# carkod/binquant

Measured on AMD Instinct MI355X. Metric: symbol-candles/s for full indicator set (14 fp64 columns), higher is better.
Workload: dtype f64; 1 GPU; configs[3]: 100000 symbols x 10000 candles, symbol-sharded over 1 GPU(s) (100000 symbols x 10000 candles on rank 0); symbols=100000, symbols_per_gpu=100000, candles=10000, parallelism=symbol-sharded x1, no data-path collective

## Files before the change

### binquant_amd/csrc/bq_context.hip

```cpp
#include "bq_context.h"
#include "binquant_amd.h"

#include <string.h>

namespace bq {

constexpr int CX_NW = 4;
constexpr int CX_NT = CX_NW * WAVE;
constexpr int CX_K = CTX_K;
constexpr int CX_TT = WAVE * CX_K;
constexpr int CX_HS = 20;
constexpr int CX_RS = CX_HS + CX_TT;
constexpr int CX_Q = CX_RS / CX_K;
static_assert(CX_HS % CX_K == 0 && CX_RS % CX_K == 0, "ring shape");
#define CXS(i) ((((i) & (CX_K - 1)) * CX_Q) + ((i) >> 2))
constexpr int CX_ATR = 14;
constexpr int CX_BB = 20;

constexpr int CNT_VALID = 0, CNT_ADV = 3, CNT_DEC = 6, CNT_A20 = 9, CNT_A50 = 12;

struct CtxArgs {
  const double* h;
  const double* l;
  const double* c;
  int64_t S, ld_in;
  int T, M;
  int vin;
  FeatEma E;
  int lag20, lag50;
  double* gsum[4];
  uint16_t* gcnt;
  int64_t ld_g;
  double* last[BQ_NUM_FEATURES];
  double* feat[BQ_NUM_FEATURES];
  int64_t ld_f;
  int vout;
};

__device__ __forceinline__ void wave_sync() {
  __builtin_amdgcn_fence(__ATOMIC_RELEASE, "wavefront");
  __builtin_amdgcn_wave_barrier();
  __builtin_amdgcn_fence(__ATOMIC_ACQUIRE, "wavefront");
}

__device__ __forceinline__ double cx_rcp(double b) { return rcp_nr(fabs(b)); }
__device__ __forceinline__ double cx_mul_rcp(double a, double b, double r) { return b < 0.0 ? -(a * r) : a * r; }
__device__ __forceinline__ double cx_div(double a, double b) { return cx_mul_rcp(a, b, cx_rcp(b)); }

template <bool DIV, bool RING, bool FEAT = false, int MC = 0>
__global__ __launch_bounds__(CX_NT, 3) void context_partials_kernel(const CtxArgs A) {
  __shared__ double sTr[CX_NW][CX_RS], sC[CX_NW][CX_RS];
  __shared__ double sR[2][4][CX_TT];
  __shared__ uint16_t sN[2][CX_TT];
  __shared__ float sD[RING ? CX_NW : 1][RING ? 3 * CX_TT : 1];

  const int lane = threadIdx.x & (WAVE - 1), w = threadIdx.x / WAVE;
  const int64_t grp = blockIdx.x;
  const int64_t sym = grp * CX_NW + w;
  const bool live = sym < A.S;
  const int64_t row = live ? sym : A.S - 1;
  const int T = A.T, M = MC > 0 ? MC : A.M;
  const double* __restrict__ rH = A.h + row * A.ld_in;
  const double* __restrict__ rL = A.l + row * A.ld_in;
  const double* __restrict__ rC = A.c + row * A.ld_in;
  double* __restrict__ trr = sTr[w];
  double* __restrict__ cr = sC[w];
  const bool vin = A.vin != 0;
  const int WB = M < CX_BB ? M : CX_BB;

  if (lane < CX_HS) {
    trr[CXS(lane)] = 0.0;
    cr[CXS(lane)] = qnan();
  }
  double c1c = qnan(), c2c = qnan(), hc = qnan(), lc = qnan();
  int rcC = -1, rtC = -1;
  double ecar[2] = {0.0, 0.0}, lcar[2] = {0.0, 0.0};
  double lpow[2], rpow[2];
#pragma unroll
  for (int e = 0; e < 2; ++e) {
    lpow[e] = pow_bits<6>(A.E.apow[e], lane);
    rpow[e] = pow_bits<5>(A.E.apow[e], (lane & 15) + 1);
  }
  wave_sync();

  for (int t0 = 0; t0 < T; t0 += CX_TT) {
    const int tb = t0 + CX_K * lane, qb = CX_HS + CX_K * lane;
    double h[CX_K], l[CX_K], c[CX_K], xl[CX_K];
    load4<double2>(rH, tb, T, vin, h);
    load4<double2>(rL, tb, T, vin, l);
    load4<double2>(rC, tb, T, vin, c);
    if (!RING && (A.lag20 || A.lag50)) {
#pragma unroll
      for (int k = 0; k < CX_K; ++k) {
        const int s = tb + k - (M - 1);
        xl[k] = (s >= 0 && s < T) ? rC[s] : 0.0;
      }
    }

    double p1 = dpp_f64<DPP_WAVE_SHR1>(c[CX_K - 1]);
    double p2 = dpp_f64<DPP_WAVE_SHR1>(c[CX_K - 2]);
    double ph = dpp_f64<DPP_WAVE_SHR1>(h[CX_K - 1]);
    double pl = dpp_f64<DPP_WAVE_SHR1>(l[CX_K - 1]);
    if (lane == 0) {
      p1 = c1c;
      p2 = c2c;
      ph = hc;
      pl = lc;
    }
    double tr[CX_K];
    int lcc[CX_K], lct[CX_K];
    {
      double pcv = p1, ptr = true_range(ph, pl, p2), cp = p1;
      int rc = -1, rt = -1;
#pragma unroll
      for (int k = 0; k < CX_K; ++k) {
        const int t = tb + k;
        tr[k] = true_range(h[k], l[k], cp);
        if (t == 0 || c[k] != pcv) rc = t;
        if (t == 0 || tr[k] != ptr) rt = t;
        lcc[k] = rc;
        lct[k] = rt;
        pcv = c[k];
        ptr = tr[k];
        cp = c[k];
      }
    }
#pragma unroll
    for (int k = 0; k < CX_K; ++k) {
      cr[CXS(qb + k)] = c[k];
      trr[CXS(qb + k)] = tr[k];
    }
    {
      const int ic = wave_scan_max_dpp(lcc[CX_K - 1] + 1, lane) - 1;
      const int it = wave_scan_max_dpp(lct[CX_K - 1] + 1, lane) - 1;
      const int a = dpp_i32<DPP_WAVE_SHR1>(ic + 1) - 1, b = dpp_i32<DPP_WAVE_SHR1>(it + 1) - 1;
      const int ec = max(lane == 0 ? -1 : a, rcC), et = max(lane == 0 ? -1 : b, rtC);
#pragma unroll
      for (int k = 0; k < CX_K; ++k) {
        lcc[k] = max(lcc[k], ec);
        lct[k] = max(lct[k], et);
      }
    }
    double Y[2][CX_K], D[2][CX_K];
#pragma unroll
    for (int e = 0; e < 2; ++e) {
      const double al = A.E.alpha[e], om = A.E.om[e], dn = A.E.den[e];
      {
        double y = 0.0;
#pragma unroll
        for (int k = 0; k < CX_K; ++k) y = (tb + k == 0) ? c[k] : fma(A.E.lin_a[e], y, A.E.lin_b[e] * c[k]);
        const double inc = wave_scan_affine_dpp_rp(y, A.E.apow[e], rpow[e], lane);
        const double ex = dpp_f64<DPP_WAVE_SHR1>(inc);
        double v = lane == 0 ? ecar[e] : fma(lpow[e], ecar[e], ex);
#pragma unroll
        for (int k = 0; k < CX_K; ++k) {
          const double x = c[k];
          if (tb + k == 0) v = x;
          else if (v != x) v = DIV ? (om * v + al * x) / dn : om * v + al * x;
          Y[e][k] = v;
        }
        ecar[e] = readlane_f64(v, WAVE - 1);
      }
      const bool lag = !RING && (e == 0 ? A.lag20 : A.lag50);
#pragma unroll
      for (int k = 0; k < CX_K; ++k) D[e][k] = 0.0;
      if (lag) {
        const int s0 = tb - (M - 1);
        double y = 0.0;
#pragma unroll
        for (int k = 0; k < CX_K; ++k) y = (s0 + k == 0) ? xl[k] : fma(A.E.lin_a[e], y, A.E.lin_b[e] * xl[k]);
        const double inc = wave_scan_affine_dpp_rp(y, A.E.apow[e], rpow[e], lane);
        const double ex = dpp_f64<DPP_WAVE_SHR1>(inc);
        double v = lane == 0 ? lcar[e] : fma(lpow[e], lcar[e], ex);
#pragma unroll
        for (int k = 0; k < CX_K; ++k) {
          const int s = s0 + k;
          const double x = xl[k];
          if (s == 0) v = x;
          else if (s > 0 && v != x) v = DIV ? (om * v + al * x) / dn : om * v + al * x;
          D[e][k] = v - x;
        }
        lcar[e] = readlane_f64(v, WAVE - 1);
      }
    }
    if (RING) {
      float* dr = sD[w];
      const int dslot = ((t0 / CX_TT) % 3) * CX_TT;
#pragma unroll
      for (int k = 0; k < CX_K; ++k) dr[dslot + CX_K * lane + k] = (float)(Y[1][k] - c[k]);
    }
    wave_sync();
    if (RING) {
      const float* dr = sD[w];
      int r = ((t0 / CX_TT) % 3) * CX_TT + CX_K * lane - (M - 1);
      r += r < 0 ? 3 * CX_TT : 0;
#pragma unroll
      for (int k = 0; k < CX_K; ++k) {
        const int q = r + k >= 3 * CX_TT ? r + k - 3 * CX_TT : r + k;
        D[1][k] = (double)dr[q];
      }
    }

    double atr[CX_K], mid[CX_K], sd[CX_K];
    if (tb >= CX_BB - 1 && WB == CX_BB) {
      {
        double a[CX_ATR - 1];
#pragma unroll
        for (int i = 0; i < CX_ATR - 1; ++i) a[i] = trr[CXS(qb - (CX_ATR - 1) + i)];
        double Sx = 0.0;
#pragma unroll
        for (int i = 0; i < CX_ATR - 1; ++i) Sx += a[i];
#pragma unroll
        for (int k = 0; k < CX_K; ++k) {
          Sx = k == 0 ? Sx + tr[0] : (Sx + tr[k]) - a[k - 1];
          atr[k] = div_count(Sx < 0.0 ? 0.0 : Sx, (double)CX_ATR, 1.0 / CX_ATR);
        }
      }
      {
        const double r = c[0];
        double d0[CX_K - 1];
        double s1 = 0.0, s2 = 0.0;
#pragma unroll
        for (int i = 0; i < CX_BB - 1; ++i) {
          const double d = cr[CXS(qb - (CX_BB - 1) + i)] - r;
          if (i < CX_K - 1) d0[i] = d;
          s1 += d;
          s2 = fma(d, d, s2);
        }
#pragma unroll
        for (int k = 0; k < CX_K; ++k) {
          const double dn = c[k] - r;
          if (k == 0) {
            s1 += dn;
            s2 = fma(dn, dn, s2);
          } else {
            const double dol = d0[k - 1];
            s1 = (s1 + dn) - dol;
            s2 = fma(-dol, dol, fma(dn, dn, s2));
          }
          const double m1 = s1 * (1.0 / CX_BB);
          const double var = fma(-m1, s1, s2) * (1.0 / CX_BB);
          mid[k] = r + m1;
          sd[k] = sqrt_nr(var > 0.0 ? var : 0.0);
        }
      }
    } else {
#pragma unroll
      for (int k = 0; k < CX_K; ++k) {
        const int t = tb + k, q = qb + k;
        const int n = min(t + 1, M);
        const int ma = min(CX_ATR, n), mb = min(WB, n);
        double Sx = 0.0;
        for (int i = q - ma + 1; i <= q; ++i) Sx += trr[CXS(i)];
        atr[k] = (Sx < 0.0 ? 0.0 : Sx) / (double)ma;
        double m = 0.0;
        for (int i = q - mb + 1; i <= q; ++i) m += cr[CXS(i)];
        m = m / (double)mb;
        double acc = 0.0;
        for (int i = q - mb + 1; i <= q; ++i) {
          const double d = cr[CXS(i)] - m;
          acc = fma(d, d, acc);
        }
        mid[k] = m;
        sd[k] = sqrt(acc / (double)mb);
      }
    }
    double fr[CX_K], fe20[CX_K], fe50[CX_K], ftr[CX_K], fap[CX_K], fbw[CX_K];
    double rc[CX_K + 1];
    rc[0] = cx_rcp(p1);
#pragma unroll
    for (int k = 0; k < CX_K; ++k) rc[k + 1] = cx_rcp(c[k]);
#pragma unroll
    for (int k = 0; k < CX_K; ++k) {
      const int t = tb + k;
      const int n = min(t + 1, M);
      if (n < 2) {
        fr[k] = fe20[k] = fe50[k] = ftr[k] = fap[k] = fbw[k] = qnan();
        continue;
      }
      const double cl = c[k];
      const double prev = k > 0 ? c[k - 1] : p1;
      double e20 = Y[0][k], e50 = Y[1][k];
      if (t + 1 > M) {
        e20 = e20 - A.E.corr[0] * D[0][k];
        e50 = e50 - A.E.corr[1] * D[1][k];
      }
      const double a = lct[k] <= t - min(CX_ATR, n) + 1 ? tr[k] : atr[k];
      double m = mid[k], s = sd[k];
      if (lcc[k] <= t - min(WB, n) + 1) {
        m = cl;
        s = 0.0;
      }
      const double up = m + (2.0 * s), lo = m - (2.0 * s);
      fr[k] = prev == 0.0 ? 0.0 : cx_mul_rcp(cl - prev, prev, rc[k]);
      fe20[k] = e20;
      fe50[k] = e50;
      ftr[k] = e50 != 0.0 ? cx_div(e20 - e50, e50 < 0.0 ? -e50 : e50) : 0.0;
      fap[k] = cl != 0.0 ? cx_mul_rcp(a, cl, rc[k + 1]) : 0.0;
      fbw[k] = m != 0.0 ? cx_div(up - lo, m < 0.0 ? -m : m) : 0.0;
    }
    if constexpr (FEAT) {
      if (live) {
        const int64_t orow = sym * A.ld_f;
        const bool vo = A.vout != 0, whole = t0 + CX_TT <= T;
        const double* const cols[BQ_NUM_FEATURES] = {fr, fe20, fe50, ftr, fap, fbw};
#pragma unroll
        for (int f = 0; f < BQ_NUM_FEATURES; ++f)
          if (A.feat[f]) {
            double v[CX_K];
#pragma unroll
            for (int k = 0; k < CX_K; ++k) v[k] = cols[f][k];
            store_lines<CX_K>(A.feat[f] + orow, tb, T, vo, v, whole);
          }
      }
    } else {
    if (live && tb <= T - 1 && T - 1 < tb + CX_K) {
#pragma unroll
      for (int k = 0; k < CX_K; ++k) {
        if (tb + k != T - 1) continue;
        const double v[BQ_NUM_FEATURES] = {fr[k], fe20[k], fe50[k], ftr[k], fap[k], fbw[k]};
#pragma unroll
        for (int f = 0; f < BQ_NUM_FEATURES; ++f)
          if (A.last[f]) A.last[f][sym] = v[f];
      }
    }

    double cs[4][CX_K];
    unsigned cn[CX_K];
#pragma unroll
    for (int k = 0; k < CX_K; ++k) {
      const double r = fr[k];
      const bool ok = live && tb + k < T && r == r;
      cn[k] = ok ? ((1u << CNT_VALID) | ((r > 0.0 ? 1u : 0u) << CNT_ADV) | ((r < 0.0 ? 1u : 0u) << CNT_DEC) |
                    ((c[k] > fe20[k] ? 1u : 0u) << CNT_A20) | ((c[k] > fe50[k] ? 1u : 0u) << CNT_A50))
                 : 0u;
      cs[0][k] = ok ? r : 0.0;
      cs[1][k] = ok ? ftr[k] : 0.0;
      cs[2][k] = ok ? fap[k] : 0.0;
      cs[3][k] = ok ? fbw[k] : 0.0;
    }
    if (w & 1) {
      const int sl = w >> 1;
#pragma unroll
      for (int k = 0; k < CX_K; ++k) {
#pragma unroll
        for (int f = 0; f < 4; ++f) sR[sl][f][k * WAVE + lane] = cs[f][k];
        sN[sl][k * WAVE + lane] = (uint16_t)cn[k];
      }
    }
    __syncthreads();
    if (!(w & 1)) {
      const int sl = w >> 1;
#pragma unroll
      for (int k = 0; k < CX_K; ++k) {
#pragma unroll
        for (int f = 0; f < 4; ++f) cs[f][k] = cs[f][k] + sR[sl][f][k * WAVE + lane];
        cn[k] += sN[sl][k * WAVE + lane];
      }
      if (w == 2) {
#pragma unroll
        for (int k = 0; k < CX_K; ++k) {
#pragma unroll
          for (int f = 0; f < 4; ++f) sR[1][f][k * WAVE + lane] = cs[f][k];
          sN[1][k * WAVE + lane] = (uint16_t)cn[k];
        }
      }
    }
    __syncthreads();
    if (w == 0) {
#pragma unroll
      for (int k = 0; k < CX_K; ++k) {
#pragma unroll
        for (int f = 0; f < 4; ++f) cs[f][k] = cs[f][k] + sR[1][f][k * WAVE + lane];
        cn[k] += sN[1][k * WAVE + lane];
      }
      const int64_t orow = grp * A.ld_g;
#pragma unroll
      for (int f = 0; f < 4; ++f) store_lines<CX_K>(A.gsum[f] + orow, tb, T, true, cs[f]);
      uint16_t* gc = A.gcnt + orow;
      if (tb + CX_K <= T) {
        const uint64_t packed = (uint64_t)cn[0] | ((uint64_t)cn[1] << 16) | ((uint64_t)cn[2] << 32) |
                                ((uint64_t)cn[3] << 48);
        __builtin_nontemporal_store(packed, reinterpret_cast<uint64_t*>(gc + tb));
      } else {
#pragma unroll
        for (int k = 0; k < CX_K; ++k)
          if (tb + k < T) gc[tb + k] = (uint16_t)cn[k];
      }
    }
    }

    if (t0 + CX_TT >= T) break;
    wave_sync();
    if (lane < CX_HS) {
      const int src = CX_TT + lane;
      trr[CXS(lane)] = trr[CXS(src)];
      cr[CXS(lane)] = cr[CXS(src)];
    }
    wave_sync();
    c1c = readlane_f64(c[CX_K - 1], WAVE - 1);
    c2c = readlane_f64(c[CX_K - 2], WAVE - 1);
    hc = readlane_f64(h[CX_K - 1], WAVE - 1);
    lc = readlane_f64(l[CX_K - 1], WAVE - 1);
    rcC = __builtin_amdgcn_readlane(lcc[CX_K - 1], WAVE - 1);
    rtC = __builtin_amdgcn_readlane(lct[CX_K - 1], WAVE - 1);
  }
}

constexpr int GR_TW = 64;
constexpr int GR_NW = 4;
constexpr int GR_U = 8;
constexpr int CX_NSUM = 9;

struct GroupReduceArgs {
  const double* gsum[4];
  const uint16_t* gcnt;
  int64_t ngrp, ld_g, per_chunk;
  int T;
  double* chunk;
};

__global__ __launch_bounds__(GR_TW * GR_NW) void context_group_reduce_kernel(const GroupReduceArgs A) {
  __shared__ double sAcc[GR_NW][CX_NSUM][GR_TW + 1];
  const int lane = threadIdx.x & (WAVE - 1), u = threadIdx.x / WAVE;
  const int t = blockIdx.x * GR_TW + lane;
  const int64_t g0 = (int64_t)blockIdx.y * A.per_chunk;
  const int64_t g1 = min(A.ngrp, g0 + A.per_chunk);
  double s[4] = {0.0, 0.0, 0.0, 0.0};
  int n[5] = {0, 0, 0, 0, 0};
  auto add = [&](const double (&v)[4], unsigned c) {
#pragma unroll
    for (int f = 0; f < 4; ++f) s[f] += v[f];
    n[0] += (c >> CNT_VALID) & 7u;
    n[1] += (c >> CNT_ADV) & 7u;
    n[2] += (c >> CNT_DEC) & 7u;
    n[3] += (c >> CNT_A20) & 7u;
    n[4] += (c >> CNT_A50) & 7u;
  };
  if (t < A.T) {
    int64_t g = g0 + u;
    for (; g + (GR_U - 1) * GR_NW < g1; g += GR_U * GR_NW) {
      double v[GR_U][4];
      unsigned c[GR_U];
#pragma unroll
      for (int j = 0; j < GR_U; ++j) {
        const int64_t o = (g + j * GR_NW) * A.ld_g + t;
#pragma unroll
        for (int f = 0; f < 4; ++f) v[j][f] = A.gsum[f][o];
        c[j] = A.gcnt[o];
      }
#pragma unroll
      for (int j = 0; j < GR_U; ++j) add(v[j], c[j]);
    }
    for (; g < g1; g += GR_NW) {
      const int64_t o = g * A.ld_g + t;
      double v[4];
#pragma unroll
      for (int f = 0; f < 4; ++f) v[f] = A.gsum[f][o];
      add(v, A.gcnt[o]);
    }
  }
#pragma unroll
  for (int i = 0; i < 5; ++i) sAcc[u][i][lane] = (double)n[i];
#pragma unroll
  for (int f = 0; f < 4; ++f) sAcc[u][5 + f][lane] = s[f];
  __syncthreads();
  if (u == 0 && t < A.T) {
    double acc[CX_NSUM];
#pragma unroll
    for (int i = 0; i < CX_NSUM; ++i) acc[i] = sAcc[0][i][lane];
    for (int v = 1; v < GR_NW; ++v)
#pragma unroll
      for (int i = 0; i < CX_NSUM; ++i) acc[i] += sAcc[v][i][lane];
    double* o = A.chunk + ((int64_t)blockIdx.y * A.T + t) * CX_NSUM;
#pragma unroll
    for (int i = 0; i < CX_NSUM; ++i) o[i] = acc[i];
  }
}

__global__ __launch_bounds__(256) void context_chunk_reduce_kernel(const double* __restrict__ chunk, int nchunk, int T,
                                                                   double* __restrict__ partial) {
  const int t = blockIdx.x * 256 + threadIdx.x;
  if (t >= T) return;
  double acc[CX_NSUM];
#pragma unroll
  for (int i = 0; i < CX_NSUM; ++i) acc[i] = 0.0;
  for (int j = 0; j < nchunk; ++j) {
    const double* c = chunk + ((int64_t)j * T + t) * CX_NSUM;
#pragma unroll
    for (int i = 0; i < CX_NSUM; ++i) acc[i] += c[i];
  }
  double* o = partial + (int64_t)t * BQ_NUM_PARTIALS;
#pragma unroll
  for (int i = 0; i < CX_NSUM; ++i) o[i] = acc[i];
  o[BQ_P_RESERVED] = 0.0;
}

struct CtxLayout {
  int64_t ngrp, ld_g, nchunk, per_chunk;
  size_t off_sum[4], off_cnt, off_chunk, bytes;
};

static size_t align256(size_t x) { return (x + 255) & ~(size_t)255; }

static CtxLayout ctx_layout(int64_t S, int64_t T) {
  CtxLayout L;
  L.ngrp = (S + CX_NW - 1) / CX_NW;
  L.ld_g = (T + 63) & ~(int64_t)63;
  const int64_t tblocks = (T + GR_TW - 1) / GR_TW;
  int64_t nch = (2048 + tblocks - 1) / (tblocks > 0 ? tblocks : 1);
  nch = nch < 1 ? 1 : nch;
  const int64_t maxch = (L.ngrp + 3) / 4;
  if (nch > maxch) nch = maxch < 1 ? 1 : maxch;
  L.per_chunk = (L.ngrp + nch - 1) / nch;
  L.nchunk = (L.ngrp + L.per_chunk - 1) / L.per_chunk;
  size_t o = 0;
  for (int f = 0; f < 4; ++f) {
    L.off_sum[f] = o;
    o = align256(o + (size_t)L.ngrp * L.ld_g * sizeof(double));
  }
  L.off_cnt = o;
  o = align256(o + (size_t)L.ngrp * L.ld_g * sizeof(uint16_t));
  L.off_chunk = o;
  o = align256(o + (size_t)L.nchunk * T * CX_NSUM * sizeof(double));
  L.bytes = o;
  return L;
}

static CtxArgs ctx_args(const double* const* hlc, int64_t S, int64_t T, int64_t ld_in, int max_bars) {
  CtxArgs A;
  memset(&A, 0, sizeof(A));
  A.h = hlc[0];
  A.l = hlc[1];
  A.c = hlc[2];
  A.S = S;
  A.ld_in = ld_in;
  A.T = (int)T;
  A.M = max_bars;
  A.vin = vec_rows(hlc, 3, ld_in);
  A.E = feat_ema_consts(max_bars);
  A.lag20 = A.E.corr[0] >= 1e-15;
  A.lag50 = A.E.corr[1] >= 1e-15;
  if (!A.lag20) A.E.corr[0] = 0.0;
  if (!A.lag50) A.E.corr[1] = 0.0;
  return A;
}

template <bool FEAT, bool DIV>
static void launch_context_div(const CtxArgs& A, unsigned ngrp, int max_bars, hipStream_t st) {
  const bool ring = A.E.corr[1] <= 1e-6 && !A.lag20;
  const dim3 grid(ngrp), block(CX_NT);
  if (!FEAT && ring && max_bars == 400)
    hipLaunchKernelGGL((context_partials_kernel<DIV, true, false, 400>), grid, block, 0, st, A);
  else if (ring) hipLaunchKernelGGL((context_partials_kernel<DIV, true, FEAT>), grid, block, 0, st, A);
  else hipLaunchKernelGGL((context_partials_kernel<DIV, false, FEAT>), grid, block, 0, st, A);
}

template <bool FEAT>
static void launch_context(const CtxArgs& A, unsigned ngrp, int max_bars, hipStream_t st) {
  if (A.E.den[0] != 1.0 || A.E.den[1] != 1.0) launch_context_div<FEAT, true>(A, ngrp, max_bars, st);
  else launch_context_div<FEAT, false>(A, ngrp, max_bars, st);
}

int context_features(const double* const* hlc, int64_t S, int64_t T, int64_t ld_in, int32_t max_bars,
                     double* const* feat, int64_t ld_out, hipStream_t st) {
  CtxArgs A = ctx_args(hlc, S, T, ld_in, max_bars);
  for (int f = 0; f < BQ_NUM_FEATURES; ++f) A.feat[f] = feat[f];
  A.ld_f = ld_out;
  A.vout = vec_rows(feat, BQ_NUM_FEATURES, ld_out);
  launch_context<true>(A, (unsigned)((S + CX_NW - 1) / CX_NW), max_bars, st);
  return hipGetLastError() == hipSuccess ? BQ_OK : BQ_EHIP;
}

}

extern "C" {

size_t bq_context_workspace_bytes(int64_t S, int64_t T) {
  if (S <= 0 || T <= 0) return 0;
  return bq::ctx_layout(S, T).bytes;
}

int bq_context_partials(const double* const* hlc, int64_t S, int64_t T, int64_t ld_in, int32_t max_bars,
                        void* workspace, size_t workspace_bytes, double* partial, double* const* last_feat,
                        void* stream) {
  using namespace bq;
  if (!hlc || !hlc[0] || !hlc[1] || !hlc[2] || !partial || S < 0 || T < 0 || ld_in < T || max_bars < 15 ||
      max_bars > BQ_MAX_HISTORY + 1 || T > (int64_t)0x7fffffff - CX_TT || S > (int64_t)0x7fffffff * CX_NW)
    return BQ_EINVAL;
  if (S == 0 || T == 0) {
    if (T > 0 && hipMemsetAsync(partial, 0, (size_t)T * BQ_NUM_PARTIALS * sizeof(double), (hipStream_t)stream) != hipSuccess)
      return BQ_EHIP;
    return hipGetLastError() == hipSuccess ? BQ_OK : BQ_EHIP;
  }
  const CtxLayout L = ctx_layout(S, T);
  if (!workspace || workspace_bytes < L.bytes || (((uintptr_t)workspace) & 255u)) return BQ_EINVAL;
  CtxArgs A = ctx_args(hlc, S, T, ld_in, max_bars);
  char* ws = (char*)workspace;
  for (int f = 0; f < 4; ++f) A.gsum[f] = (double*)(ws + L.off_sum[f]);
  A.gcnt = (uint16_t*)(ws + L.off_cnt);
  A.ld_g = L.ld_g;
  for (int f = 0; f < BQ_NUM_FEATURES; ++f) A.last[f] = last_feat ? last_feat[f] : nullptr;
  hipStream_t st = (hipStream_t)stream;
  launch_context<false>(A, (unsigned)L.ngrp, max_bars, st);
  GroupReduceArgs G;
  for (int f = 0; f < 4; ++f) G.gsum[f] = A.gsum[f];
  G.gcnt = A.gcnt;
  G.ngrp = L.ngrp;
  G.ld_g = L.ld_g;
  G.per_chunk = L.per_chunk;
  G.T = (int)T;
  G.chunk = (double*)(ws + L.off_chunk);
  hipLaunchKernelGGL(context_group_reduce_kernel, dim3((unsigned)((T + GR_TW - 1) / GR_TW), (unsigned)L.nchunk),
                     dim3(GR_TW * GR_NW), 0, st, G);
  hipLaunchKernelGGL(context_chunk_reduce_kernel, dim3((unsigned)((T + 255) / 256)), dim3(256), 0, st,
                     (const double*)G.chunk, (int)L.nchunk, (int)T, partial);
  return hipGetLastError() == hipSuccess ? BQ_OK : BQ_EHIP;
}

}
```

Before: 41.72 billion symbol-candles/s.

## Software-prefetch next tile of OHLC inputs across the context partials loop

Adds register double-buffering in the context partials kernel: the next tile's high/low/close values are loaded into spare registers during the cross-wave reduction, so their global-load latency overlaps with the LDS reduction and barriers. The carry-over readlanes move earlier so the prefetched registers can be reused. __syncthreads is replaced with an LDS-only fence plus s_barrier, which narrows the memory ordering to local memory. This costs extra VGPRs (12 doubles per lane) and could reduce occupancy under the launch bounds of 3.

```diff
diff --git a/binquant_amd/csrc/bq_context.hip b/binquant_amd/csrc/bq_context.hip
--- a/binquant_amd/csrc/bq_context.hip
+++ b/binquant_amd/csrc/bq_context.hip
@@ -47,6 +47,43 @@
 __device__ __forceinline__ double cx_mul_rcp(double a, double b, double r) { return b < 0.0 ? -(a * r) : a * r; }
 __device__ __forceinline__ double cx_div(double a, double b) { return cx_mul_rcp(a, b, cx_rcp(b)); }
 
+__device__ __forceinline__ void lds_barrier() {
+  __builtin_amdgcn_fence(__ATOMIC_RELEASE, "workgroup", "local");
+  __builtin_amdgcn_s_barrier();
+  __builtin_amdgcn_fence(__ATOMIC_ACQUIRE, "workgroup", "local");
+}
+
+__device__ __forceinline__ void load4_whole(const double* __restrict__ row, int tb, double (&x)[CX_K]) {
+  const double2* p = reinterpret_cast<const double2*>(row + tb);
+#pragma unroll
+  for (int j = 0; j < CX_K / 2; ++j) {
+    const double2 a = p[j];
+    x[2 * j] = a.x;
+    x[2 * j + 1] = a.y;
+  }
+}
+
+__device__ __forceinline__ void prefetch_tile(bool issue, const double* __restrict__ rH, const double* __restrict__ rL,
+                                              const double* __restrict__ rC, int tn, double (&hn)[CX_K],
+                                              double (&ln)[CX_K], double (&cn)[CX_K]) {
+  if (issue) {
+    load4_whole(rH, tn, hn);
+    load4_whole(rL, tn, ln);
+    load4_whole(rC, tn, cn);
+  } else {
+#pragma unroll
+    for (int k = 0; k < CX_K; ++k) {
+      hn[k] = 0.0;
+      ln[k] = 0.0;
+      cn[k] = 0.0;
+    }
+  }
+}
+
+#ifndef BQ_CX_PREFETCH
+#define BQ_CX_PREFETCH 2
+#endif
+
 template <bool DIV, bool RING, bool FEAT = false, int MC = 0>
 __global__ __launch_bounds__(CX_NT, 3) void context_partials_kernel(const CtxArgs A) {
   __shared__ double sTr[CX_NW][CX_RS], sC[CX_NW][CX_RS];
@@ -83,12 +120,25 @@
   }
   wave_sync();
 
+  constexpr bool PF = !FEAT && BQ_CX_PREFETCH != 0;
+  double hn[CX_K], ln[CX_K], cnx[CX_K];
   for (int t0 = 0; t0 < T; t0 += CX_TT) {
     const int tb = t0 + CX_K * lane, qb = CX_HS + CX_K * lane;
     double h[CX_K], l[CX_K], c[CX_K], xl[CX_K];
-    load4<double2>(rH, tb, T, vin, h);
-    load4<double2>(rL, tb, T, vin, l);
-    load4<double2>(rC, tb, T, vin, c);
+    if (PF && vin && t0 > 0 && t0 <= T - CX_TT) {
+#pragma unroll
+      for (int k = 0; k < CX_K; ++k) {
+        h[k] = hn[k];
+        l[k] = ln[k];
+        c[k] = cnx[k];
+      }
+    } else {
+      load4<double2>(rH, tb, T, vin, h);
+      load4<double2>(rL, tb, T, vin, l);
+      load4<double2>(rC, tb, T, vin, c);
+    }
+    const bool pfn = PF && vin && t0 <= T - 2 * CX_TT;
+    auto prefetch = [&]() { prefetch_tile(pfn, rH, rL, rC, tb + CX_TT, hn, ln, cnx); };
     if (!RING && (A.lag20 || A.lag50)) {
 #pragma unroll
       for (int k = 0; k < CX_K; ++k) {
@@ -299,6 +349,7 @@
       fap[k] = cl != 0.0 ? cx_mul_rcp(a, cl, rc[k + 1]) : 0.0;
       fbw[k] = m != 0.0 ? cx_div(up - lo, m < 0.0 ? -m : m) : 0.0;
     }
+    double c1n, c2n, hcn, lcn;
     if constexpr (FEAT) {
       if (live) {
         const int64_t orow = sym * A.ld_f;
@@ -325,6 +376,7 @@
       }
     }
 
+    if (BQ_CX_PREFETCH == 1) prefetch();
     double cs[4][CX_K];
     unsigned cn[CX_K];
 #pragma unroll
@@ -339,6 +391,13 @@
       cs[2][k] = ok ? fap[k] : 0.0;
       cs[3][k] = ok ? fbw[k] : 0.0;
     }
+    if (PF) {
+      c1n = readlane_f64(c[CX_K - 1], WAVE - 1);
+      c2n = readlane_f64(c[CX_K - 2], WAVE - 1);
+      hcn = readlane_f64(h[CX_K - 1], WAVE - 1);
+      lcn = readlane_f64(l[CX_K - 1], WAVE - 1);
+    }
+    if (BQ_CX_PREFETCH == 2) prefetch();
     if (w & 1) {
       const int sl = w >> 1;
 #pragma unroll
@@ -348,7 +407,8 @@
         sN[sl][k * WAVE + lane] = (uint16_t)cn[k];
       }
     }
-    __syncthreads();
+    lds_barrier();
+    if (BQ_CX_PREFETCH == 3) prefetch();
     if (!(w & 1)) {
       const int sl = w >> 1;
 #pragma unroll
@@ -366,7 +426,7 @@
         }
       }
     }
-    __syncthreads();
+    lds_barrier();
     if (w == 0) {
 #pragma unroll
       for (int k = 0; k < CX_K; ++k) {
@@ -398,10 +458,17 @@
       cr[CXS(lane)] = cr[CXS(src)];
     }
     wave_sync();
-    c1c = readlane_f64(c[CX_K - 1], WAVE - 1);
-    c2c = readlane_f64(c[CX_K - 2], WAVE - 1);
-    hc = readlane_f64(h[CX_K - 1], WAVE - 1);
-    lc = readlane_f64(l[CX_K - 1], WAVE - 1);
+    if (PF) {
+      c1c = c1n;
+      c2c = c2n;
+      hc = hcn;
+      lc = lcn;
+    } else {
+      c1c = readlane_f64(c[CX_K - 1], WAVE - 1);
+      c2c = readlane_f64(c[CX_K - 2], WAVE - 1);
+      hc = readlane_f64(h[CX_K - 1], WAVE - 1);
+      lc = readlane_f64(l[CX_K - 1], WAVE - 1);
+    }
     rcC = __builtin_amdgcn_readlane(lcc[CX_K - 1], WAVE - 1);
     rtC = __builtin_amdgcn_readlane(lct[CX_K - 1], WAVE - 1);
   }
```

After: 41.73 billion symbol-candles/s (median of 3 runs). Within noise of the previous version (+0.0%).
